# JohnsonLabJanelia/laserCalib

Hardware: AMD Instinct MI355X
Metric: LM iters/sec and residual+Jacobian Mobs/s at 16 cams x 50k points (higher is better)
Workload: dtype f32; 1 GPU; 16 cams x 50000 points per GPU, full visibility, 11-parameter cameras (800000 obs per GPU, 800000 total), full on-device Schur-complement LM iteration; cams=16, points_per_gpu=50000, camera_parameters=11, observations_total=800000, parallelism=points sharded x1, cameras replicated, collectives=none

## Files before the change

### lasercalib_amd/csrc/sba_chol_blocked.hpp

```cpp
#pragma once
#include "sba_lm_kernels.hpp"

namespace SBA_NS {

constexpr int CB = 16;
constexpr int CLD = 17;
constexpr int CBS = CB * CLD;
constexpr int CHOLB_THREADS = 512;
constexpr int CHOLB_LDS_THREADS = 512;
constexpr int CHOLB_MAX_NB = 11;

__device__ inline int cb_off(int r, int c) { return (r * (r + 1) / 2 + c) * CBS; }

__device__ inline double readlane_f64(double v, int src) {
  const int lo = __builtin_amdgcn_readlane(__double2loint(v), src);
  const int hi = __builtin_amdgcn_readlane(__double2hiint(v), src);
  return __hiloint2double(hi, lo);
}
__device__ inline double rsqrt_nr(double x) {
  const double y = __builtin_amdgcn_rsq(x);
  return y * (1.5 - 0.5 * x * y * y);
}

template <bool NEWTON = true>
__device__ __forceinline__ bool chol16_wave(double* __restrict__ blk) {
  const int lane = threadIdx.x & 63;
  const int i = lane & 15;
  const bool ident = lane >= 16;
  double a[CB];
#pragma unroll
  for (int j = 0; j < CB; ++j) { const double v = blk[i * CLD + j]; a[j] = ident ? ((j == i) ? 1.0 : 0.0) : v; }
  double dg = blk[i * CLD + i];
  __builtin_amdgcn_wave_barrier();
  auto pivot = [](double x) { return NEWTON ? rsqrt_nr(x) : __builtin_amdgcn_rsq(x); };
  double akk = readlane_f64(dg, 0);
  double piv = pivot(akk);
  double chk = piv;
#pragma unroll
  for (int k = 0; k < CB; ++k) {
    const double lik = a[k] * piv;
    a[k] = lik;
    if (k + 1 < CB) {
      dg = __builtin_fma(-lik, lik, dg);
      akk = readlane_f64(dg, k + 1);
      piv = pivot(akk);
      chk += piv;
    }
#pragma unroll
    for (int j = k + 1; j < CB; ++j) a[j] -= lik * readlane_f64(lik, j);
  }
  if (lane >= 16 && lane < 32) {
#pragma unroll
    for (int j = 0; j < CB; ++j) blk[i * CLD + j] = a[j];
  }
  return isfinite(chk) && chk > 0.0;
}

__device__ __forceinline__ void chol_panel_block(double* __restrict__ Ablk, const double* __restrict__ LinvT) {
  const int lane = threadIdx.x & 63;
  const double* Pa = Ablk + (lane & 15) * CLD + (lane >> 4);
  const double* Pl = LinvT + (lane >> 4) * CLD + (lane & 15);
  Mfma<double>::acc_t acc = {0, 0, 0, 0};
#pragma unroll
  for (int ks = 0; ks < 4; ++ks) acc = Mfma<double>::mma(Pa[4 * ks], Pl[4 * ks * CLD], acc);
  __builtin_amdgcn_wave_barrier();
#pragma unroll
  for (int rg = 0; rg < 4; ++rg) Ablk[((lane >> 4) + 4 * rg) * CLD + (lane & 15)] = acc[rg];
  __builtin_amdgcn_wave_barrier();
}

__device__ __forceinline__ void chol_update_tile(double* __restrict__ Dt, const double* __restrict__ Pa_blk, const double* __restrict__ Pb_blk) {
  const int lane = threadIdx.x & 63;
  const double* Pa = Pa_blk + (lane & 15) * CLD + (lane >> 4);
  const double* Pb = Pb_blk + (lane & 15) * CLD + (lane >> 4);
  Mfma<double>::acc_t acc, prod = {0, 0, 0, 0};
#pragma unroll
  for (int rg = 0; rg < 4; ++rg) acc[rg] = Dt[((lane >> 4) + 4 * rg) * CLD + (lane & 15)];
#pragma unroll
  for (int ks = 0; ks < 4; ++ks) prod = Mfma<double>::mma(Pa[4 * ks], Pb[4 * ks], prod);
#pragma unroll
  for (int rg = 0; rg < 4; ++rg) Dt[((lane >> 4) + 4 * rg) * CLD + (lane & 15)] = acc[rg] - prod[rg];
  __builtin_amdgcn_wave_barrier();
}

__device__ __forceinline__ void chol_update_tile2(double* __restrict__ Dt0, const double* __restrict__ Pa0_blk, const double* __restrict__ Pb0_blk,
                                                  double* __restrict__ Dt1, const double* __restrict__ Pa1_blk, const double* __restrict__ Pb1_blk) {
  const int lane = threadIdx.x & 63;
  const int po = (lane & 15) * CLD + (lane >> 4);
  double a0[4], b0[4], a1[4], b1[4];
#pragma unroll
  for (int ks = 0; ks < 4; ++ks) { a0[ks] = Pa0_blk[po + 4 * ks]; b0[ks] = Pb0_blk[po + 4 * ks]; }
#pragma unroll
  for (int ks = 0; ks < 4; ++ks) { a1[ks] = Pa1_blk[po + 4 * ks]; b1[ks] = Pb1_blk[po + 4 * ks]; }
  Mfma<double>::acc_t acc0, acc1, p0 = {0, 0, 0, 0}, p1 = {0, 0, 0, 0};
#pragma unroll
  for (int rg = 0; rg < 4; ++rg) { acc0[rg] = Dt0[((lane >> 4) + 4 * rg) * CLD + (lane & 15)]; acc1[rg] = Dt1[((lane >> 4) + 4 * rg) * CLD + (lane & 15)]; }
#pragma unroll
  for (int ks = 0; ks < 4; ++ks) { p0 = Mfma<double>::mma(a0[ks], b0[ks], p0); p1 = Mfma<double>::mma(a1[ks], b1[ks], p1); }
#pragma unroll
  for (int rg = 0; rg < 4; ++rg) Dt0[((lane >> 4) + 4 * rg) * CLD + (lane & 15)] = acc0[rg] - p0[rg];
#pragma unroll
  for (int rg = 0; rg < 4; ++rg) Dt1[((lane >> 4) + 4 * rg) * CLD + (lane & 15)] = acc1[rg] - p1[rg];
  __builtin_amdgcn_wave_barrier();
}

__device__ __forceinline__ void chol_panel_update_diag(double* __restrict__ Pblk, const double* __restrict__ LinvT, double* __restrict__ Dt) {
  const int lane = threadIdx.x & 63;
  const double* Pa = Pblk + (lane & 15) * CLD + (lane >> 4);
  const double* Pl = LinvT + (lane >> 4) * CLD + (lane & 15);
  Mfma<double>::acc_t d;
#pragma unroll
  for (int rg = 0; rg < 4; ++rg) d[rg] = Dt[((lane >> 4) + 4 * rg) * CLD + (lane & 15)];
  Mfma<double>::acc_t pt = {0, 0, 0, 0};
#pragma unroll
  for (int ks = 0; ks < 4; ++ks) pt = Mfma<double>::mma(Pl[4 * ks * CLD], Pa[4 * ks], pt);
  __builtin_amdgcn_wave_barrier();
  Mfma<double>::acc_t pp = {0, 0, 0, 0};
#pragma unroll
  for (int ks = 0; ks < 4; ++ks) pp = Mfma<double>::mma(pt[ks], pt[ks], pp);
#pragma unroll
  for (int rg = 0; rg < 4; ++rg) d[rg] -= pp[rg];
#pragma unroll
  for (int rg = 0; rg < 4; ++rg) Pblk[(lane & 15) * CLD + (lane >> 4) + 4 * rg] = pt[rg];
#pragma unroll
  for (int rg = 0; rg < 4; ++rg) Dt[((lane >> 4) + 4 * rg) * CLD + (lane & 15)] = d[rg];
  __builtin_amdgcn_wave_barrier();
}

template <typename S> struct CholNum;
template <> struct CholNum<double> {
  static constexpr int LD = CLD, BS = CB * LD;
  static __device__ __forceinline__ int off(int r, int c) { return (r * (r + 1) / 2 + c) * BS; }
  static __device__ __forceinline__ double fma(double a, double b, double c) { return __builtin_fma(a, b, c); }
  static __device__ __forceinline__ double bcast(double v, int src) { return readlane_f64(v, src); }
  static __device__ __forceinline__ double rsq(double x) { return __builtin_amdgcn_rsq(x); }
  static __device__ __forceinline__ double xrow(double v) { return xrow_sum(v); }
};
template <> struct CholNum<float> {
  static constexpr int LD = 20, BS = CB * LD;
  static __device__ __forceinline__ int off(int r, int c) { return (r * (r + 1) / 2 + c) * BS; }
  static __device__ __forceinline__ float fma(float a, float b, float c) { return __builtin_fmaf(a, b, c); }
  static __device__ __forceinline__ float bcast(float v, int src) { return __int_as_float(__builtin_amdgcn_readlane(__float_as_int(v), src)); }
  static __device__ __forceinline__ float rsq(float x) { return __builtin_amdgcn_rsqf(x); }
  static __device__ __forceinline__ float xrow(float v) {
    unsigned a0 = __float_as_uint(v), a1 = a0;
    asm volatile("s_nop 1\n\tv_permlane16_swap_b32 %0, %1\n\ts_nop 1" : "+v"(a0), "+v"(a1));
    const float p = __uint_as_float(a0) + __uint_as_float(a1);
    a0 = __float_as_uint(p); a1 = a0;
    asm volatile("s_nop 1\n\tv_permlane32_swap_b32 %0, %1\n\ts_nop 1" : "+v"(a0), "+v"(a1));
    return __uint_as_float(a0) + __uint_as_float(a1);
  }
};

template <typename S, int LDV = CholNum<S>::LD> struct CholLay {
  static constexpr int LD = LDV, BS = CB * LDV;
  static __device__ __forceinline__ int off(int r, int c) { return (r * (r + 1) / 2 + c) * BS; }
};

template <typename S, bool NEWTON, typename L = CholLay<S>>
__device__ __forceinline__ bool chol16_wave_t(S* __restrict__ blk, const S* __restrict__ a0 = nullptr, S tau = (S)0) {
  const int lane = threadIdx.x & 63;
  const int i = lane & 15;
  const bool ident = lane >= 16;
  S a[CB];
#pragma unroll
  for (int j = 0; j < CB; ++j) { const S v = blk[i * L::LD + j]; a[j] = ident ? ((j == i) ? (S)1 : (S)0) : v; }
  S dg = blk[i * L::LD + i];
  __builtin_amdgcn_wave_barrier();
  auto pivot = [](S x) -> S {
    if constexpr (NEWTON) return (S)rsqrt_nr((double)x);
    else return CholNum<S>::rsq(x);
  };
  S akk = CholNum<S>::bcast(dg, 0);
  S piv = pivot(akk);
  S chk = piv;
#pragma unroll
  for (int k = 0; k < CB; ++k) {
    const S lik = a[k] * piv;
    a[k] = lik;
    if (k + 1 < CB) {
      dg = CholNum<S>::fma(-lik, lik, dg);
      akk = CholNum<S>::bcast(dg, k + 1);
      piv = pivot(akk);
      chk += piv;
    }
#pragma unroll
    for (int j = k + 1; j < CB; ++j) a[j] -= lik * CholNum<S>::bcast(lik, j);
  }
  if (lane >= 16 && lane < 32) {
#pragma unroll
    for (int j = 0; j < CB; ++j) blk[i * L::LD + j] = a[j];
  }
  bool ok = isfinite(chk) && chk > (S)0;
  if (a0) {
    __builtin_amdgcn_wave_barrier();
    const S li = blk[i * L::LD + i];
    const bool sunk = lane < 16 && !(((S)1 / (li * li)) >= tau * a0[i]);
    ok = ok && !__any(sunk);
  }
  return ok;
}

template <typename S, typename L = CholLay<S>>
__device__ __forceinline__ void chol_panel_block_t(S* __restrict__ Ablk, const S* __restrict__ LinvT) {
  const int lane = threadIdx.x & 63;
  const S* Pa = Ablk + (lane & 15) * L::LD + (lane >> 4);
  const S* Pl = LinvT + (lane >> 4) * L::LD + (lane & 15);
  typename Mfma<S>::acc_t acc = {0, 0, 0, 0};
#pragma unroll
  for (int ks = 0; ks < 4; ++ks) acc = Mfma<S>::mma(Pa[4 * ks], Pl[4 * ks * L::LD], acc);
  __builtin_amdgcn_wave_barrier();
#pragma unroll
  for (int rg = 0; rg < 4; ++rg) Ablk[Mfma<S>::row_of(lane, rg) * L::LD + (lane & 15)] = acc[rg];
  __builtin_amdgcn_wave_barrier();
}

template <typename S, typename L = CholLay<S>>
__device__ __forceinline__ void chol_panel_update_diag_t(S* __restrict__ Pblk, const S* __restrict__ LinvT, S* __restrict__ Dt) {
  const int lane = threadIdx.x & 63;
  const S* Pa = Pblk + (lane & 15) * L::LD + (lane >> 4);
  const S* Pl = LinvT + (lane >> 4) * L::LD + (lane & 15);
  typename Mfma<S>::acc_t d;
#pragma unroll
  for (int rg = 0; rg < 4; ++rg) d[rg] = Dt[Mfma<S>::row_of(lane, rg) * L::LD + (lane & 15)];
  typename Mfma<S>::acc_t pt = {0, 0, 0, 0};
#pragma unroll
  for (int ks = 0; ks < 4; ++ks) pt = Mfma<S>::mma(Pl[4 * ks * L::LD], Pa[4 * ks], pt);
  __builtin_amdgcn_wave_barrier();
  typename Mfma<S>::acc_t pp = {0, 0, 0, 0};
#pragma unroll
  for (int ks = 0; ks < 4; ++ks) pp = Mfma<S>::mma(pt[ks], pt[ks], pp);
#pragma unroll
  for (int rg = 0; rg < 4; ++rg) d[rg] -= pp[rg];
#pragma unroll
  for (int rg = 0; rg < 4; ++rg) Pblk[(lane & 15) * L::LD + Mfma<S>::row_of(lane, rg)] = pt[rg];
#pragma unroll
  for (int rg = 0; rg < 4; ++rg) Dt[Mfma<S>::row_of(lane, rg) * L::LD + (lane & 15)] = d[rg];
  __builtin_amdgcn_wave_barrier();
}

template <int MAXNB> struct CholbShared {
  int fail;
  short rc[MAXNB * (MAXNB + 1) / 2];
  double dd[MAXNB * CB];
  double x[MAXNB * CB];
};
template <int MAXNB> struct CholbPre {
  static constexpr int BPR = CHOLB_LDS_THREADS / 128;
  static constexpr int U0 = (MAXNB + BPR - 1) / BPR;
  static constexpr int NREM = MAXNB * (MAXNB - 1) / 2;
  static constexpr int TREM = CHOLB_LDS_THREADS - 64;
  static constexpr int U1_ALL = (NREM * 128 + TREM - 1) / TREM;
  static constexpr int U1 = U1_ALL < 16 ? U1_ALL : 16;
};

__device__ __forceinline__ void lds_barrier() { asm volatile("s_waitcnt lgkmcnt(0)\n\ts_barrier" ::: "memory"); }

template <int MAXNB, int LD> struct CholbImg {
  static_assert((CB * LD) % 4 == 0, "a block is a whole number of 16-byte pieces");
  static constexpr int NBE = (MAXNB > CHOLB_MAX_NB && LD == 20) ? 14 : MAXNB;
  static constexpr int F4B = CB * LD / 4;
  static constexpr int R0 = (NBE * F4B + CHOLB_LDS_THREADS - 1) / CHOLB_LDS_THREADS;
  static constexpr int TREM = CHOLB_LDS_THREADS - 64;
  static constexpr int R1 = (NBE * (NBE - 1) / 2 * F4B + TREM - 1) / TREM;
};
template <int MAXNB, int LD> struct CholbImgRegs {
  float4 q0[CholbImg<MAXNB, LD>::R0];
  float4 q1[CholbImg<MAXNB, LD>::R1];
  int m1[CholbImg<MAXNB, LD>::R1];
};
template <int LD> __device__ __forceinline__ int cholb_img_diag(int w) {
  const int p0 = 4 * w, row = (p0 + 3) / (LD + 1), pd = row * (LD + 1);
  return (pd >= p0 && row < CB) ? ((row + 1) | ((pd - p0) << 8)) : 0;
}
__device__ __forceinline__ void cholb_img_patch(float4& v, int comp, float d) {
  v.x = comp == 0 ? d : v.x; v.y = comp == 1 ? d : v.y; v.z = comp == 2 ? d : v.z; v.w = comp == 3 ? d : v.w;
}

template <typename S, bool NEWTON, int LOAD, int MAXNB, typename L = CholLay<S>>
__device__ __forceinline__ bool cholb_core(unsigned char* __restrict__ smem, CholbShared<MAXNB>& sh, const double* __restrict__ E, const int n,
                                           double (&c0)[CholbPre<MAXNB>::U0][2], double (&c1)[CholbPre<MAXNB>::U1][2], const int (&rc1)[CholbPre<MAXNB>::U1],
                                           const S tau, long long* __restrict__ dbg, int& nstamp,
                                           CholbImgRegs<MAXNB, L::LD>* __restrict__ img = nullptr) {
#define CHOL_STAMP() do { if (dbg && threadIdx.x == 0) dbg[nstamp] = clock64(); ++nstamp; } while (0)
  using Pre = CholbPre<MAXNB>;
  constexpr int BPR = Pre::BPR, U0 = Pre::U0, TREM = Pre::TREM, U1 = Pre::U1;
  constexpr bool F32 = std::is_same<S, float>::value;
  const int tid = threadIdx.x, lane = tid & 63, wid = tid >> 6;
  const int nb = (n + CB - 1) / CB;
  const int n16 = nb * CB;
  const int nblk = nb * (nb + 1) / 2;
  S* Lb = reinterpret_cast<S*>(smem);
  S* s_y = Lb + nblk * L::BS;
  S* s_a0 = s_y + n16;
  const int s4 = tid >> 7, ii0 = (tid >> 3) & 15, jp0 = tid & 7;
  auto fix = [&](int I, int J, double& v0, double& v1) {
    if (I >= n || J >= n) v0 = (I == J) ? 1.0 : 0.0;
    if (I >= n || J + 1 >= n) v1 = (I == J + 1) ? 1.0 : 0.0;
  };
  if (tid < n16) s_y[tid] = (S)sh.x[tid];
  if constexpr (LOAD == 2) {
    using Im = CholbImg<MAXNB, L::LD>;
    float4* Lb4 = reinterpret_cast<float4*>(smem);
#pragma unroll
    for (int u = 0; u < Im::R0; ++u) {
      const int e = tid + CHOLB_LDS_THREADS * u;
      if (e < nb * Im::F4B) {
        const int r = e / Im::F4B, w = e - r * Im::F4B;
        float4 v = img->q0[u];
        const int dg = (r == 0) ? cholb_img_diag<L::LD>(w) : 0;
        if (dg) cholb_img_patch(v, dg >> 8, s_a0[(dg & 255) - 1]);
        Lb4[(r * (r + 1) / 2) * Im::F4B + w] = v;
      }
    }
    lds_barrier();
    CHOL_STAMP();
    if (wid > 0) {
#pragma unroll
      for (int u = 0; u < Im::R1; ++u) {
        const int e = (tid - 64) + Im::TREM * u;
        if (e < (nblk - nb) * Im::F4B) {
          const int m = img->m1[u], g = (m >> 16) & 0x1ff;
          float4 v = img->q1[u];
          if (g) cholb_img_patch(v, (m >> 28) & 3, s_a0[g - 1]);
          Lb4[m & 0xffff] = v;
        }
      }
    }
  } else if constexpr (LOAD == 1) {
#pragma unroll
    for (int u = 0; u < U0; ++u) fix((BPR * u + s4) * CB + ii0, 2 * jp0, c0[u][0], c0[u][1]);
    {
      const int ii = ii0, jp = jp0;
#pragma unroll
      for (int u = 0; u < U0; ++u) {
        const int r = BPR * u + s4;
        if (r < nb) {
          const int I = r * CB + ii, J = 2 * jp;
          S* dst = Lb + L::off(r, 0) + ii * L::LD + J;
          const double v0 = c0[u][0] + ((I == J && I < n) ? sh.dd[I] : 0.0), v1 = c0[u][1] + ((I == J + 1 && I < n) ? sh.dd[I] : 0.0);
          dst[0] = (S)v0;
          dst[1] = (S)v1;
          if (F32 && I == J) s_a0[I] = (S)v0;
          if (F32 && I == J + 1) s_a0[I] = (S)v1;
        }
      }
    }
    __syncthreads();
    CHOL_STAMP();
    if (wid > 0) {
#pragma unroll
      for (int u = 0; u < U1; ++u) {
        const int e = (tid - 64) + TREM * u;
        if (e < (nblk - nb) * 128) {
          const int rc = rc1[u];
          const int br = rc >> 8, bc = rc & 255;
          const int ii = (e >> 3) & 15, I = br * CB + ii, J = bc * CB + 2 * (e & 7);
          S* dst = Lb + L::off(br, bc) + ii * L::LD + 2 * (e & 7);
          fix(I, J, c1[u][0], c1[u][1]);
          double d0 = 0.0, d1 = 0.0;
          if (br == bc) {
            d0 = (I == J && I < n) ? sh.dd[I] : 0.0;
            d1 = (I == J + 1 && I < n) ? sh.dd[I] : 0.0;
          }
          dst[0] = (S)(c1[u][0] + d0);
          dst[1] = (S)(c1[u][1] + d1);
          if (F32 && br == bc && I == J) s_a0[I] = (S)(c1[u][0] + d0);
          if (F32 && br == bc && I == J + 1) s_a0[I] = (S)(c1[u][1] + d1);
        }
      }
      if constexpr (Pre::U1 < Pre::U1_ALL) {
        const int first = U1 * TREM, last = (nblk - nb) * 128;
        for (int e0 = first + (tid - 64); e0 < last; e0 += 4 * TREM) {
          double v[4][2];
          int rcq[4];
#pragma unroll
          for (int q = 0; q < 4; ++q) {
            const int e = min(e0 + q * TREM, last - 1);
            const int k = e >> 7;
            int cc = 1, base = 0;
            while (k >= base + (nb - cc) && cc < nb) { base += nb - cc; ++cc; }
            rcq[q] = ((cc + (k - base)) << 8) | cc;
            const int I = (cc + (k - base)) * CB + ((e >> 3) & 15), J = cc * CB + 2 * (e & 7);
            const double* qp = E + (size_t)min(I, n - 1) * n + min(J, n - 1);
            v[q][0] = qp[0]; v[q][1] = qp[(J + 1 < n && I < n) ? 1 : 0];
          }
#pragma unroll
          for (int q = 0; q < 4; ++q) {
            const int e = e0 + q * TREM;
            if (e < last) {
              const int br = rcq[q] >> 8, bc = rcq[q] & 255;
              const int ii = (e >> 3) & 15, I = br * CB + ii, J = bc * CB + 2 * (e & 7);
              S* dst = Lb + L::off(br, bc) + ii * L::LD + 2 * (e & 7);
              fix(I, J, v[q][0], v[q][1]);
              double d0 = 0.0, d1 = 0.0;
              if (br == bc) { d0 = (I == J && I < n) ? sh.dd[I] : 0.0; d1 = (I == J + 1 && I < n) ? sh.dd[I] : 0.0; }
              dst[0] = (S)(v[q][0] + d0);
              dst[1] = (S)(v[q][1] + d1);
              if (F32 && br == bc && I == J) s_a0[I] = (S)(v[q][0] + d0);
              if (F32 && br == bc && I == J + 1) s_a0[I] = (S)(v[q][1] + d1);
            }
          }
        }
      }
    }
  } else {
    for (int e = tid; e < nblk * CB * CB; e += CHOLB_LDS_THREADS) {
      const int k = e >> 8, rc = sh.rc[k], br = rc >> 8, bc = rc & 255;
      const int ii = (e >> 4) & 15, jj = e & 15, I = br * CB + ii, J = bc * CB + jj;
      double v = (I < n && J < n) ? E[(size_t)I * n + J] : ((I == J) ? 1.0 : 0.0);
      if (I == J && I < n) v += sh.dd[I];
      Lb[L::off(br, bc) + ii * L::LD + jj] = (S)v;
      if (F32 && I == J) s_a0[I] = (S)v;
    }
    __syncthreads();
    CHOL_STAMP();
  }
  if (wid == 0) {
    if (!chol16_wave_t<S, NEWTON, L>(Lb + L::off(0, 0), F32 ? s_a0 : nullptr, tau)) { if (lane == 0) sh.fail = 1; }
  }
  __syncthreads();
  CHOL_STAMP();

  constexpr int NW = CHOLB_LDS_THREADS / 64;
  for (int jb = 0; jb < nb && !sh.fail; ++jb) {
    const int m = (nb - jb - 1) * CB;
    const S* LinvT = Lb + L::off(jb, jb);
    if (wid == 0) {
      if (jb + 1 < nb) chol_panel_update_diag_t<S, L>(Lb + L::off(jb + 1, jb), LinvT, Lb + L::off(jb + 1, jb + 1));
    } else {
      for (int r = jb + 2 + (wid - 1); r < nb; r += NW - 1) chol_panel_block_t<S, L>(Lb + L::off(r, jb), LinvT);
      if (wid == NW - 1) {
        const int i = lane & 15, part = lane >> 4;
        S x = 0;
#pragma unroll
        for (int kk = 0; kk < 4; ++kk) { const int k = part + 4 * kk; x += LinvT[k * L::LD + i] * s_y[jb * CB + k]; }
        x = CholNum<S>::xrow(x);
        __builtin_amdgcn_wave_barrier();
        if (part == 0) s_y[jb * CB + i] = x;
      }
    }
    __syncthreads();
    CHOL_STAMP();
    if (wid == 0) {
      if (jb + 1 < nb) {
        if (!chol16_wave_t<S, NEWTON, L>(Lb + L::off(jb + 1, jb + 1), F32 ? s_a0 + (jb + 1) * CB : nullptr, tau)) { if (lane == 0) sh.fail = 1; }
      }
    } else {
      if (wid == 4) {
        for (int t = lane; t < m; t += 64) {
          const S* row = Lb + L::off(jb + 1 + (t >> 4), jb) + (t & 15) * L::LD;
          S s0 = 0, s1 = 0;
#pragma unroll
          for (int k = 0; k < CB; k += 2) { s0 += row[k] * s_y[jb * CB + k]; s1 += row[k + 1] * s_y[jb * CB + k + 1]; }
          s_y[(jb + 1) * CB + t] -= s0 + s1;
        }
      } else {
        constexpr int NWORK = NW - 2;
        const int wk = wid - 1 - (wid > 4 ? 1 : 0);
        const int q = nb - jb - 1;
        const int ntile = q * (q + 1) / 2;
        const int per = (ntile - 1 + NWORK - 1) / NWORK;
        int t = 1 + wk * per;
        const int t_hi = min(ntile, t + per);
        if (t < t_hi) {
          const int rc = sh.rc[t];
          int r = jb + 1 + (rc >> 8), c = jb + 1 + (rc & 255);
          const int po = (lane & 15) * L::LD + (lane >> 4);
          const int to = Mfma<S>::row_of(lane, 0) * L::LD + (lane & 15);
          constexpr int trs = F32 ? L::LD : 4 * L::LD;
          while (t < t_hi) {
            const S* Ap = Lb + L::off(r, jb) + po;
            S a[4];
#pragma unroll
            for (int ks = 0; ks < 4; ++ks) a[ks] = Ap[4 * ks];
            S* D = Lb + L::off(r, c) + to;
            const S* Bp = Lb + L::off(c, jb) + po;
            for (; c <= r && t < t_hi; ++c, ++t) {
              S bq[4];
#pragma unroll
              for (int ks = 0; ks < 4; ++ks) bq[ks] = Bp[4 * ks];
              typename Mfma<S>::acc_t acc, prod = {0, 0, 0, 0};
#pragma unroll
              for (int rg = 0; rg < 4; ++rg) acc[rg] = D[rg * trs];
#pragma unroll
              for (int ks = 0; ks < 4; ++ks) prod = Mfma<S>::mma(a[ks], bq[ks], prod);
#pragma unroll
              for (int rg = 0; rg < 4; ++rg) D[rg * trs] = acc[rg] - prod[rg];
              D += L::BS;
              Bp += (c + 1) * L::BS;
            }
            ++r;
            c = jb + 1;
          }
          __builtin_amdgcn_wave_barrier();
        }
      }
    }
    if (dbg && jb == 0 && lane == 0) dbg[40 + wid] = clock64();
    __syncthreads();
    CHOL_STAMP();
  }
  const bool fail = sh.fail != 0;
  if (!fail) {
    for (int b = nb - 1; b >= 0; --b) {
      if (wid == 0) {
        const int j = lane & 15, part = lane >> 4;
        const S* LiT = Lb + L::off(b, b) + j * L::LD;
        S x = 0;
#pragma unroll
        for (int ii = 0; ii < 4; ++ii) { const int i = part + 4 * ii; x += LiT[i] * s_y[b * CB + i]; }
        x = CholNum<S>::xrow(x);
        __builtin_amdgcn_wave_barrier();
        if (part == 0) s_y[b * CB + j] = x;
      }
      __syncthreads();
      if (tid < b * CB) {
        const S* col = Lb + L::off(b, tid >> 4) + (tid & 15);
        S s0 = 0, s1 = 0;
#pragma unroll
        for (int i = 0; i < CB; i += 2) { s0 += col[i * L::LD] * s_y[b * CB + i]; s1 += col[(i + 1) * L::LD] * s_y[b * CB + i + 1]; }
        s_y[tid] -= s0 + s1;
      }
      __syncthreads();
    }
    if (tid < n16) sh.x[tid] = (double)s_y[tid];
  }
  __syncthreads();
  CHOL_STAMP();
  return fail;
#undef CHOL_STAMP
}

template <typename T, int MAXNB = CHOLB_MAX_NB, int LD32 = 20, bool IMG = false>
__global__ __launch_bounds__(CHOLB_LDS_THREADS) void k_cholesky_blocked(
    const double* __restrict__ E , int C,
    LMState* __restrict__ st, double* __restrict__ D2c, const ParamSets<T> ps,
    double* __restrict__ delta_c, int n_sys ,
    const int32_t* __restrict__ tie ,
    const int32_t* __restrict__ first ,
    long long* __restrict__ dbg , int use_f32, float tau32,
    const float* __restrict__ img ) {
  extern __shared__ __align__(16) unsigned char smem[];
  static_assert(!IMG || std::is_same<T, float>::value, "the f32 image exists for the fp32 engine only");
  constexpr bool PIV_NEWTON = !std::is_same<T, float>::value;
  const int n = n_sys;
  const int tid = threadIdx.x, lane = tid & 63, wid = tid >> 6;
  const double* rhs = E + (size_t)n * n;
  const double* dU = rhs + n;
  const double* gct = dU + n;
  const bool pair_ok = (n & 1) == 0;
  using Pre = CholbPre<MAXNB>;
  using L32 = CholLay<float, LD32>;
  constexpr int BPR = Pre::BPR, U0 = Pre::U0, TREM = Pre::TREM, U1 = Pre::U1;
  double c0[U0][2];
  const int nlast = n - 1;
  auto addr = [&](int I, int J) { return E + (size_t)min(I, nlast) * n + min(J, nlast - 1 + (pair_ok ? 0 : 1)); };
  const int s4 = tid >> 7, ii0 = (tid >> 3) & 15, jp0 = tid & 7;
  const int tclamp = min(tid, nlast);
  using Im = CholbImg<MAXNB, LD32>;
  CholbImgRegs<MAXNB, LD32> ir;
  const float4* img4 = reinterpret_cast<const float4*>(img);
  const int nb_ = (n + CB - 1) / CB;
  if constexpr (IMG) {
#pragma unroll
    for (int u = 0; u < Im::R0; ++u) {
      const int e = min(tid + CHOLB_LDS_THREADS * u, nb_ * Im::F4B - 1);
      const int r = e / Im::F4B;
      ir.q0[u] = img4[(r * (r + 1) / 2) * Im::F4B + (e - r * Im::F4B)];
    }
  } else if (pair_ok) {
#pragma unroll
    for (int u = 0; u < U0; ++u) {
      const double2 t = *reinterpret_cast<const double2*>(addr((BPR * u + s4) * CB + ii0, 2 * jp0));
      c0[u][0] = t.x; c0[u][1] = t.y;
    }
  } else {
#pragma unroll
    for (int u = 0; u < U0; ++u) {
      const double* q = addr((BPR * u + s4) * CB + ii0, 2 * jp0);
      c0[u][0] = q[0]; c0[u][1] = q[(2 * jp0 + 1 < n) ? 1 : 0];
    }
  }
  double in_d = D2c[tclamp], in_u = dU[tclamp], in_r = rhs[tclamp];
  const double my_g = (tid < n) ? gct[tid] : 0.0;
  double in_e = 0.0;
  if constexpr (IMG) in_e = E[(size_t)tclamp * n + tclamp];
  double c1[U1][2];
  int rc1[U1];
  if constexpr (IMG) {
    const int last = max((nb_ * (nb_ + 1) / 2 - nb_) * Im::F4B - 1, 0);
    int rr = 1, base = 0;
#pragma unroll
    for (int u = 0; u < Im::R1; ++u) {
      const int e = min(max(tid - 64, 0) + Im::TREM * u, last);
      const int k = e / Im::F4B, w = e - k * Im::F4B;
      while (k >= base + rr && rr < nb_) { base += rr; ++rr; }
      const int f = (k + rr + 1) * Im::F4B + w;
      const int dg = (k - base + 1 == rr) ? cholb_img_diag<LD32>(w) : 0;
      ir.m1[u] = f | (dg ? (((rr * CB + (dg & 255)) << 16) | ((dg >> 8) << 28)) : 0);
      ir.q1[u] = img4[f];
    }
  } else {
    const int last = (nb_ * (nb_ + 1) / 2 - nb_) * 128 - 1;
    int cc = 1, base = 0;
#pragma unroll
    for (int u = 0; u < U1; ++u) {
      const int e = min(max(tid - 64, 0) + TREM * u, last);
      const int k = e >> 7;
      while (k >= base + (nb_ - cc) && cc < nb_) { base += nb_ - cc; ++cc; }
      rc1[u] = ((cc + (k - base)) << 8) | cc;
      const int I = (cc + (k - base)) * CB + ((e >> 3) & 15), J = cc * CB + 2 * (e & 7);
      if (pair_ok) {
        const double2 t = *reinterpret_cast<const double2*>(addr(I, J));
        c1[u][0] = t.x; c1[u][1] = t.y;
      } else {
        const double* q = addr(I, J);
        c1[u][0] = q[0]; c1[u][1] = q[(J + 1 < n) ? 1 : 0];
      }
    }
  }
  if (st->status >= 0) return;
  const int cur_ = ps_cur(ps, st);
  const double* __restrict__ cams = ps.cams[cur_];
  double* __restrict__ cams_new = ps.cams[cur_ ^ 1];
  T* __restrict__ campre_new = ps.campre[cur_ ^ 1];
  int nstamp = 0;
#define CHOL_STAMP() do { if (dbg && threadIdx.x == 0) dbg[nstamp] = clock64(); ++nstamp; } while (0)
  CHOL_STAMP();
  const int ncam = C * NCP;
  const int nb = (n + CB - 1) / CB;
  const int n16 = nb * CB;
  const int nblk = nb * (nb + 1) / 2;
  __shared__ CholbShared<MAXNB> sh;
  __shared__ double s_scr[4][CHOLB_LDS_THREADS / 64];
  const double lam = st->lam;
  const bool fresh = st->fresh != 0;
  const double my_cam = (tid < ncam) ? cams[tid] : 0.0;
  const double my_xs = (tid < n) ? cams[(!IMG && first) ? first[tid] : tid] : 0.0;

  if (tid < nblk) {
    int r = 0;
    while ((r + 1) * (r + 2) / 2 <= tid) ++r;
    sh.rc[tid] = (short)((r << 8) | (tid - r * (r + 1) / 2));
  }
  if (tid == 0) { sh.fail = 0; st->cost = E[(size_t)n * n + 3 * n]; }
  if (tid < n16) {
    double dd = 0;
    if (tid >= n) in_r = 0;
    if (tid < n) {
      double d = in_d;
      if (fresh) { d = fmax(d, in_u); D2c[tid] = d; }
      dd = lam * fmax_pos(d);
    }
    sh.x[tid] = in_r;
    sh.dd[tid] = dd;
    if constexpr (IMG) (reinterpret_cast<float*>(smem) + nblk * L32::BS + n16)[tid] = (float)((tid < n ? in_e : 1.0) + dd);
  }
  if constexpr (IMG) lds_barrier();
  else __syncthreads();
  bool fail;
  if constexpr (MAXNB > CHOLB_MAX_NB) {
    static_assert(std::is_same<T, float>::value, "the 16-block-row kernel exists for the fp32 engine only");
    fail = cholb_core<float, false, IMG ? 2 : 1, MAXNB, L32>(smem, sh, E, n, c0, c1, rc1, tau32, dbg, nstamp, &ir);
    if (tid == 0) { st->chol_retry = fail ? 1 : 0; if (fail) st->chol_f64_retries += 1; }
    if (fail) return;
  } else if constexpr (std::is_same<T, float>::value) {
    if (use_f32 || IMG) {
      fail = cholb_core<float, false, IMG ? 2 : 1, MAXNB, L32>(smem, sh, E, n, c0, c1, rc1, tau32, dbg, nstamp, &ir);
      if (fail) {
        __syncthreads();
        if (tid == 0) sh.fail = 0;
        __syncthreads();
        fail = cholb_core<double, true, false, MAXNB>(smem, sh, E, n, c0, c1, rc1, 0.0, dbg, nstamp);
        if (tid == 0) atomicAdd(&st->chol_f64_retries, 1);
      }
    } else if constexpr (!IMG) {
      fail = cholb_core<double, PIV_NEWTON, true, MAXNB>(smem, sh, E, n, c0, c1, rc1, 0.0, dbg, nstamp);
    }
  } else {
    fail = cholb_core<double, PIV_NEWTON, true, MAXNB>(smem, sh, E, n, c0, c1, rc1, 0.0, dbg, nstamp);
  }
  double pred = 0, dx2 = 0, x2 = 0, gm = 0;
  __shared__ double s_cnew[CHOLB_LDS_THREADS];
  if (tid < ncam) {
    const double d = fail ? 0.0 : sh.x[(!IMG && tie) ? tie[tid] : tid];
    delta_c[tid] = d;
    cams_new[tid] = my_cam + d;
    s_cnew[tid] = my_cam + d;
  }
  if (tid < n) {
    const double d = fail ? 0.0 : sh.x[tid];
    pred = 0.5 * d * (sh.dd[tid] * d - my_g);
    dx2 = d * d;
    x2 = my_xs * my_xs;
    gm = fabs(my_g);
  }
  pred = wave_sum(pred); dx2 = wave_sum(dx2); x2 = wave_sum(x2); gm = wave_max(gm);
  if (lane == 0) { s_scr[0][wid] = pred; s_scr[1][wid] = dx2; s_scr[2][wid] = x2; s_scr[3][wid] = gm; }
  __syncthreads();
  if (tid == 0) {
    double p = 0, d2 = 0, xx = 0, g = 0;
    for (int w = 0; w < CHOLB_LDS_THREADS / 64; ++w) { p += s_scr[0][w]; d2 += s_scr[1][w]; xx += s_scr[2][w]; g = fmax(g, s_scr[3][w]); }
    st->pred_c = p; st->dx2_c = d2; st->x2_c = xx; st->gmax_c = g;
    st->chol_fail = fail ? 1 : 0;
    st->fresh = 0;
  }
  if (tid >= 64 && tid < 64 + C)
    campre_build<T>(s_cnew + (size_t)(tid - 64) * NCP, campre_new + (size_t)(tid - 64) * CAMPRE);
  CHOL_STAMP();
#undef CHOL_STAMP
}

constexpr int CS_MAX_NB = 32;
__device__ inline size_t cs_blk(int r, int c) { return ((size_t)r * (r + 1) / 2 + c) * (CB * CB); }

__global__ __launch_bounds__(CHOLB_THREADS) void k_cholesky_stream(
    const double* __restrict__ A, int n, double* __restrict__ W ,
    double* __restrict__ sol, int* __restrict__ info, const LMState* __restrict__ st,
    int scap ,
    long long* __restrict__ dbg ) {
  extern __shared__ __align__(16) unsigned char smem[];
  if (st->status >= 0) return;
  const int nb = (n + CB - 1) / CB, n16 = nb * CB;
  double* P = reinterpret_cast<double*>(smem);
  double* S = P + (size_t)nb * CBS;
  double* s_y = S + (size_t)scap * CBS;
  __shared__ int s_fail;
  __shared__ double s_part[32][CB];
  __shared__ int s_src[72];
  const int tid = threadIdx.x, lane = tid & 63, wid = tid >> 6;
  constexpr int NW = CHOLB_THREADS / 64;
  for (int i = tid; i < n16; i += CHOLB_THREADS) s_y[i] = (i < n) ? sol[i] : 0.0;
  if (tid == 0) s_fail = 0;
  __syncthreads();
  constexpr int MAXPRE = CS_MAX_NB * CB * CB / CHOLB_THREADS;
  double pre[MAXPRE];
  auto fetch_panel = [&](int jc) {
    const int mm = nb - jc;
#pragma unroll
    for (int u = 0; u < MAXPRE; ++u) {
      const int e = tid + u * CHOLB_THREADS;
      pre[u] = 0;
      if (e < mm * CB * CB) {
        const int i = e >> 8, ii = (e >> 4) & 15, jj = e & 15;
        const int I = (jc + i) * CB + ii, J = jc * CB + jj;
        pre[u] = (I < n && J < n) ? A[(size_t)I * n + J] : ((I == J) ? 1.0 : 0.0);
      }
    }
  };
  auto fetch_column = [&](int bc) {
    const int mm = nb - bc;
#pragma unroll
    for (int u = 0; u < MAXPRE; ++u) {
      const int e = tid + u * CHOLB_THREADS;
      pre[u] = 0;
      if (e < mm * CB * CB) pre[u] = W[cs_blk(bc + (e >> 8), bc) + (e & 255)];
    }
  };
  auto commit = [&](double* dst, int mm) {
#pragma unroll
    for (int u = 0; u < MAXPRE; ++u) {
      const int e = tid + u * CHOLB_THREADS;
      if (e < mm * CB * CB) dst[(e >> 8) * CBS + ((e >> 4) & 15) * CLD + (e & 15)] = pre[u];
    }
  };
  long long ph[5] = {0, 0, 0, 0, 0}, t_prev = clock64();
  auto lap = [&](int k) { const long long t = clock64(); ph[k] += t - t_prev; t_prev = t; };
  fetch_panel(0);
  for (int j = 0; j < nb && !s_fail; ++j) {
    const int m = nb - j;
    commit(P, m);
    const int gmax = max(1, scap / m);
    for (int k0 = 0; k0 < j; k0 += gmax) {
      const int g = min(gmax, j - k0);
      __syncthreads();
      if (tid < g * m) { const int kk = tid / m, i = tid - kk * m; s_src[tid] = (int)cs_blk(j + i, k0 + kk); }
      __syncthreads();
      {
        const int tot = g * m * CB * CB;
        for (int e0 = tid; e0 < tot; e0 += 8 * CHOLB_THREADS) {
          double v[8];
#pragma unroll
          for (int u = 0; u < 8; ++u) {
            const int e = e0 + u * CHOLB_THREADS;
            v[u] = (e < tot) ? W[s_src[e >> 8] + (e & 255)] : 0.0;
          }
#pragma unroll
          for (int u = 0; u < 8; ++u) {
            const int e = e0 + u * CHOLB_THREADS;
            if (e < tot) S[(e >> 8) * CBS + ((e >> 4) & 15) * CLD + (e & 15)] = v[u];
          }
        }
      }
      __syncthreads();
      for (int i = wid; i < m; i += NW) {
        double* Dt = P + i * CBS;
        Mfma<double>::acc_t acc;
#pragma unroll
        for (int rg = 0; rg < 4; ++rg) acc[rg] = Dt[((lane >> 4) + 4 * rg) * CLD + (lane & 15)];
        Mfma<double>::acc_t acc1 = {0, 0, 0, 0};
        const int po = (lane & 15) * CLD + (lane >> 4);
        int kk = 0;
        for (; kk + 1 < g; kk += 2) {
          const double* Pa0 = S + (kk * m + i) * CBS + po;
          const double* Pb0 = S + (kk * m) * CBS + po;
          const double* Pa1 = S + ((kk + 1) * m + i) * CBS + po;
          const double* Pb1 = S + ((kk + 1) * m) * CBS + po;
          double a0[4], b0[4], a1[4], b1[4];
#pragma unroll
          for (int ks = 0; ks < 4; ++ks) { a0[ks] = Pa0[4 * ks]; b0[ks] = Pb0[4 * ks]; a1[ks] = Pa1[4 * ks]; b1[ks] = Pb1[4 * ks]; }
#pragma unroll
          for (int ks = 0; ks < 4; ++ks) {
            acc = Mfma<double>::mma(-a0[ks], b0[ks], acc);
            acc1 = Mfma<double>::mma(-a1[ks], b1[ks], acc1);
          }
        }
        if (kk < g) {
          const double* Pa = S + (kk * m + i) * CBS + po;
          const double* Pb = S + (kk * m) * CBS + po;
#pragma unroll
          for (int ks = 0; ks < 4; ++ks) acc = Mfma<double>::mma(-Pa[4 * ks], Pb[4 * ks], acc);
        }
#pragma unroll
        for (int rg = 0; rg < 4; ++rg) acc[rg] += acc1[rg];
#pragma unroll
        for (int rg = 0; rg < 4; ++rg) Dt[((lane >> 4) + 4 * rg) * CLD + (lane & 15)] = acc[rg];
      }
    }
    __syncthreads();
    lap(0);
    if (j + 1 < nb) fetch_panel(j + 1);
    if (wid == 0) {
      if (!chol16_wave(P)) { if (lane == 0) s_fail = 1; }
    }
    lds_barrier();
    lap(1);
    if (s_fail) break;
    for (int i = 1 + wid; i < m; i += NW) chol_panel_block(P + i * CBS, P);
    if (wid == NW - 1) {
      const int i = lane & 15, part = lane >> 4;
      double x = 0;
#pragma unroll
      for (int kk = 0; kk < 4; ++kk) { const int k = part + 4 * kk; x += P[k * CLD + i] * s_y[j * CB + k]; }
      x = xrow_sum(x);
      __builtin_amdgcn_wave_barrier();
      if (part == 0) s_y[j * CB + i] = x;
    }
    lds_barrier();
    lap(2);
    for (int t = tid; t < (m - 1) * CB; t += CHOLB_THREADS) {
      const double* row = P + (1 + (t >> 4)) * CBS + (t & 15) * CLD;
      double s0 = 0, s1 = 0;
#pragma unroll
      for (int k = 0; k < CB; k += 2) { s0 += row[k] * s_y[j * CB + k]; s1 += row[k + 1] * s_y[j * CB + k + 1]; }
      s_y[(j + 1) * CB + t] -= s0 + s1;
    }
    for (int e = tid; e < m * CB * CB; e += CHOLB_THREADS) {
      const int i = e >> 8, ii = (e >> 4) & 15, jj = e & 15;
      W[cs_blk(j + i, j) + ii * CB + jj] = P[i * CBS + ii * CLD + jj];
    }
    __syncthreads();
    lap(3);
  }
  __syncthreads();
  const bool fail = s_fail != 0;
  if (!fail) {
    fetch_column(nb - 1);
    for (int b = nb - 1; b >= 0; --b) {
      const int m = nb - b;
      commit(S, m);
      __syncthreads();
      if (b > 0) fetch_column(b - 1);
      {
        const int jcol = tid & 15, part = tid >> 4;
        double s0 = 0;
        for (int rr = part; rr < (m - 1) * CB; rr += 32)
          s0 += S[(1 + (rr >> 4)) * CBS + (rr & 15) * CLD + jcol] * s_y[(b + 1) * CB + rr];
        s_part[part][jcol] = s0;
      }
      __syncthreads();
      if (wid == 0) {
        const int jcol = lane & 15, part = lane >> 4;
        if (lane < CB) {
          double v = 0;
#pragma unroll
          for (int q = 0; q < 32; ++q) v += s_part[q][lane];
          s_y[b * CB + lane] -= v;
        }
        __builtin_amdgcn_wave_barrier();
        const double* LiT = S + jcol * CLD;
        double x = 0;
#pragma unroll
        for (int ii = 0; ii < 4; ++ii) { const int i = part + 4 * ii; x += LiT[i] * s_y[b * CB + i]; }
        x = xrow_sum(x);
        __builtin_amdgcn_wave_barrier();
        if (part == 0) s_y[b * CB + jcol] = x;
      }
      __syncthreads();
    }
  }
  lap(4);
  if (dbg && tid == 0) { for (int k = 0; k < 5; ++k) dbg[k] = ph[k]; }
  for (int i = tid; i < n; i += CHOLB_THREADS) sol[i] = fail ? 0.0 : s_y[i];
  if (tid == 0) *info = fail ? 1 : 0;
}

}
```

Measured before the change: 7634 Mobs/s (observations x LM iterations per second, whole job).

## Factor 16x16 diagonal Cholesky tiles with 4-wide MFMA blocked updates in f32

Adds a new f32 16x16 Cholesky-and-inverse routine that processes the tile in four 4-column groups. Each group is factored with readlane broadcasts and rsq, then the trailing matrix and the inverse are updated with 16x16x4 MFMA rank-4 updates, using permlane16/32 swaps to move panel data between lanes. The goal is to shorten the serial per-column dependency chain of the diagonal-block factorization on wave 0, which lies on the critical path of the blocked Schur solve. It drops Newton refinement of rsq, which may reduce accuracy, and it depends on gfx950-specific permlane swap instructions.

```diff
diff --git a/lasercalib_amd/csrc/sba_chol16_block4.hpp b/lasercalib_amd/csrc/sba_chol16_block4.hpp
--- /dev/null
+++ b/lasercalib_amd/csrc/sba_chol16_block4.hpp
@@ -0,0 +1,109 @@
+#pragma once
+#include <hip/hip_runtime.h>
+#include <type_traits>
+
+namespace sba_block4 {
+
+using acc4 = __attribute__((ext_vector_type(4))) float;
+
+__device__ __forceinline__ float rl(float v, int src) { return __int_as_float(__builtin_amdgcn_readlane(__float_as_int(v), src)); }
+
+struct SwapMove {
+template <int S>
+static __device__ __forceinline__ void run(float*, float v0, float v1, float v2, float v3, float z0, float z1, float z2, float z3,
+                                           float& vb, float& zb) {
+  unsigned a = __float_as_uint(v0), b = __float_as_uint(v1), c = __float_as_uint(v2), d = __float_as_uint(v3);
+  unsigned e = __float_as_uint(z0), f = __float_as_uint(z1), g = __float_as_uint(z2), h = __float_as_uint(z3);
+  asm volatile("s_nop 1\n\t"
+               "v_permlane16_swap_b32 %0, %1\n\t"
+               "v_permlane16_swap_b32 %2, %3\n\t"
+               "v_permlane16_swap_b32 %4, %5\n\t"
+               "v_permlane16_swap_b32 %6, %7\n\t"
+               "s_nop 1"
+               : "+v"(a), "+v"(b), "+v"(c), "+v"(d), "+v"(e), "+v"(f), "+v"(g), "+v"(h));
+  unsigned x = (S & 1) ? b : a, y = (S & 1) ? d : c, zx = (S & 1) ? f : e, zy = (S & 1) ? h : g;
+  asm volatile("s_nop 1\n\t"
+               "v_permlane32_swap_b32 %0, %1\n\t"
+               "v_permlane32_swap_b32 %2, %3\n\t"
+               "s_nop 1"
+               : "+v"(x), "+v"(y), "+v"(zx), "+v"(zy));
+  vb = __uint_as_float(S < 2 ? x : y);
+  zb = __uint_as_float(S < 2 ? zx : zy);
+}
+};
+
+template <int LD, typename Move = SwapMove>
+__device__ __forceinline__ bool chol16_block4_f32(float* __restrict__ blk, const float* __restrict__ a0, float tau) {
+  const int lane = threadIdx.x & 63, g = lane >> 4, c = lane & 15;
+  acc4 C, T;
+#pragma unroll
+  for (int rg = 0; rg < 4; ++rg) {
+    const int r = 4 * g + rg;
+    C[rg] = blk[max(r, c) * LD + min(r, c)];
+    T[rg] = (r == c) ? 1.0f : 0.0f;
+  }
+  __builtin_amdgcn_wave_barrier();
+  float chk = 0.0f;
+  float pv = 1.0f;
+  auto group = [&](auto sc) {
+    constexpr int s = decltype(sc)::value;
+    const int src = 20 * s;
+    float d00 = rl(C[0], src), d10 = rl(C[1], src), d20 = rl(C[2], src), d30 = rl(C[3], src);
+    float d11 = rl(C[1], src + 1), d21 = rl(C[2], src + 1), d31 = rl(C[3], src + 1);
+    float d22 = rl(C[2], src + 2), d32 = rl(C[3], src + 2);
+    float d33 = rl(C[3], src + 3);
+    const float p0 = __builtin_amdgcn_rsqf(d00);
+    const float l10 = d10 * p0, l20 = d20 * p0, l30 = d30 * p0;
+    d11 = __builtin_fmaf(-l10, l10, d11);
+    const float p1 = __builtin_amdgcn_rsqf(d11);
+    d21 = __builtin_fmaf(-l20, l10, d21);
+    d31 = __builtin_fmaf(-l30, l10, d31);
+    d22 = __builtin_fmaf(-l20, l20, d22);
+    d32 = __builtin_fmaf(-l30, l20, d32);
+    d33 = __builtin_fmaf(-l30, l30, d33);
+    const float l21 = d21 * p1, l31 = d31 * p1;
+    d22 = __builtin_fmaf(-l21, l21, d22);
+    const float p2 = __builtin_amdgcn_rsqf(d22);
+    d32 = __builtin_fmaf(-l31, l21, d32);
+    d33 = __builtin_fmaf(-l31, l31, d33);
+    const float l32 = d32 * p2;
+    d33 = __builtin_fmaf(-l32, l32, d33);
+    const float p3 = __builtin_amdgcn_rsqf(d33);
+    chk += (p0 + p1) + (p2 + p3);
+    pv = (c == 4 * s) ? p0 : pv; pv = (c == 4 * s + 1) ? p1 : pv; pv = (c == 4 * s + 2) ? p2 : pv; pv = (c == 4 * s + 3) ? p3 : pv;
+    const float z0 = T[0] * p0;
+    const float z1 = __builtin_fmaf(-l10, z0, T[1]) * p1;
+    const float z2 = __builtin_fmaf(-l21, z1, __builtin_fmaf(-l20, z0, T[2])) * p2;
+    const float z3 = __builtin_fmaf(-l32, z2, __builtin_fmaf(-l31, z1, __builtin_fmaf(-l30, z0, T[3]))) * p3;
+    if (g == s) { T[0] = z0; T[1] = z1; T[2] = z2; T[3] = z3; }
+    if constexpr (s < 3) {
+      const float v0 = C[0] * p0;
+      const float v1 = __builtin_fmaf(-l10, v0, C[1]) * p1;
+      const float v2 = __builtin_fmaf(-l21, v1, __builtin_fmaf(-l20, v0, C[2])) * p2;
+      const float v3 = __builtin_fmaf(-l32, v2, __builtin_fmaf(-l31, v1, __builtin_fmaf(-l30, v0, C[3]))) * p3;
+      float vb, zb;
+      Move::template run<s>(blk, v0, v1, v2, v3, z0, z1, z2, z3, vb, zb);
+      const float na = (c >= 4 * s + 4) ? -vb : 0.0f;
+      C = __builtin_amdgcn_mfma_f32_16x16x4f32(na, vb, C, 0, 0, 0);
+      T = __builtin_amdgcn_mfma_f32_16x16x4f32(na, zb, T, 0, 0, 0);
+    }
+  };
+  group(std::integral_constant<int, 0>{});
+  group(std::integral_constant<int, 1>{});
+  group(std::integral_constant<int, 2>{});
+  group(std::integral_constant<int, 3>{});
+  if constexpr (LD % 4 == 0) {
+    *reinterpret_cast<float4*>(blk + c * LD + 4 * g) = make_float4(T[0], T[1], T[2], T[3]);
+  } else {
+#pragma unroll
+    for (int rg = 0; rg < 4; ++rg) blk[c * LD + 4 * g + rg] = T[rg];
+  }
+  bool ok = isfinite(chk) && chk > 0.0f;
+  if (a0) {
+    const bool sunk = lane < 16 && !((1.0f / (pv * pv)) >= tau * a0[c]);
+    ok = ok && !__any(sunk);
+  }
+  return ok;
+}
+
+}
diff --git a/lasercalib_amd/csrc/sba_chol_blocked.hpp b/lasercalib_amd/csrc/sba_chol_blocked.hpp
--- a/lasercalib_amd/csrc/sba_chol_blocked.hpp
+++ b/lasercalib_amd/csrc/sba_chol_blocked.hpp
@@ -1,5 +1,6 @@
 #pragma once
 #include "sba_lm_kernels.hpp"
+#include "sba_chol16_block4.hpp"
 
 namespace SBA_NS {
 
@@ -199,6 +200,12 @@
     ok = ok && !__any(sunk);
   }
   return ok;
+}
+
+template <typename S, bool NEWTON, typename L = CholLay<S>>
+__device__ __forceinline__ bool chol16_tile(S* __restrict__ blk, const S* __restrict__ a0, S tau) {
+  if constexpr (std::is_same<S, float>::value) return sba_block4::chol16_block4_f32<L::LD>(blk, a0, tau);
+  else return chol16_wave_t<S, NEWTON, L>(blk, a0, tau);
 }
 
 template <typename S, typename L = CholLay<S>>
@@ -417,7 +424,7 @@
     CHOL_STAMP();
   }
   if (wid == 0) {
-    if (!chol16_wave_t<S, NEWTON, L>(Lb + L::off(0, 0), F32 ? s_a0 : nullptr, tau)) { if (lane == 0) sh.fail = 1; }
+    if (!chol16_tile<S, NEWTON, L>(Lb + L::off(0, 0), F32 ? s_a0 : nullptr, tau)) { if (lane == 0) sh.fail = 1; }
   }
   __syncthreads();
   CHOL_STAMP();
@@ -444,7 +451,7 @@
     CHOL_STAMP();
     if (wid == 0) {
       if (jb + 1 < nb) {
-        if (!chol16_wave_t<S, NEWTON, L>(Lb + L::off(jb + 1, jb + 1), F32 ? s_a0 + (jb + 1) * CB : nullptr, tau)) { if (lane == 0) sh.fail = 1; }
+        if (!chol16_tile<S, NEWTON, L>(Lb + L::off(jb + 1, jb + 1), F32 ? s_a0 + (jb + 1) * CB : nullptr, tau)) { if (lane == 0) sh.fail = 1; }
       }
     } else {
       if (wid == 4) {
```

Measured after the change: 7753 Mobs/s (observations x LM iterations per second, whole job) (median of 6 runs). 1.02x the previous value.
